# sile/libflate

Measured on AMD Instinct MI355X. Metric: gzip encode+decode throughput on 256 MiB synthetic text per GPU (uncompressed bytes through the round trip), higher is better.
Workload: dtype u8; 1 GPU; cfg2: gzip::Encoder (DefaultLz77Encoder, default options, mtime=0) + gzip::Decoder on TEXT(268435456 B) per GPU, write schedule S8K (8192-byte writes); bytes_per_gpu=268435456, schedule=S8K, compressed_bytes=129579521, parallelism=1 rank

## Files before the change

libflate_amd/csrc/lfx_api.cpp:

```cpp
#include "../../include/lfx.h"
#include "../../include/lfx_testhooks.h"

#include <hip/hip_runtime.h>

#include <algorithm>
#include <cstddef>
#include <cstdio>
#include <cstdlib>
#include <cstring>
#include <mutex>
#include <string>
#include <vector>

#include "lfx_ctx.h"
#include "lfx_device.h"
#include "lfx_huff.h"
#include "lfx_index.h"
#include "lfx_plan.h"
#include "lfx_abi_guard.h"

using namespace lfx;

static uint32_t host_crc32(const uint8_t *p, size_t n) {
    static uint32_t tab[256];
// ... 324 lines not shown
    hipStream_t st = c->stream;
    c->n_ev = 0;
    c->phase("start");
    for (const ChunkDesc &ch : plan.chunks)
        if (ch.len >= (1ull << 32) - 4) {
            c->set_error("an LZ77 chunk of 4 GiB or more is outside the reference's domain (u32 positions, default.rs:78)");
            return LFX_E_ARG;
        }
    const uint32_t nchunks = (uint32_t)plan.chunks.size(), nblocks = (uint32_t)plan.blocks.size();
    const bool match_v1 = c->force_match_v1 || c->diag.match_v1;
    if (c->force_match_v1 && !hc) c->match_fallbacks++;
    std::vector<SegDesc> segs;
    if (!hc) {
        uint64_t seg_len = SEG_POSITIONS;
        for (;;) {
            uint64_t cnt = 0;
            for (const ChunkDesc &ch : plan.chunks)
                if (!(ch.flags & CH_LITERALS) && ch.len > 3) cnt += div_up(ch.len - 3, seg_len);
            if (cnt >= 512 || seg_len <= 32768) break;
            seg_len /= 2;
        }
        for (uint32_t ci = 0; ci < nchunks; ci++) {
            const ChunkDesc &ch = plan.chunks[ci];
            if (ch.flags & CH_LITERALS) continue;
            for (uint64_t s = 0; s + 3 < ch.len; s += seg_len)
                segs.push_back(SegDesc{ci, (uint32_t)s, (uint32_t)std::min<uint64_t>(seg_len, ch.len - s), 0});
        }
    }
    uint64_t lnk_units = 0;
    for (SegDesc &sg : segs) {
        if (lnk_units > 0xFFFFFFFFull) { c->set_error("input too large for the link scratch"); return LFX_E_ARG; }
        sg.lnk_base = (uint32_t)lnk_units;
        lnk_units += div_up((uint64_t)sg.len + std::min<uint64_t>(sg.start, MAX_WINDOW) + 4, 64);
        lnk_units = (lnk_units + 1) & ~1ull;
    }
    std::vector<ParseWg> pwgs;
    for (uint32_t ci = 0; ci < nchunks && !hc; ci++) {
        const ChunkDesc &ch = plan.chunks[ci];
        if (ch.flags & CH_LITERALS) continue;
        for (uint32_t s = 0; s < ch.n_seg; s += PARSE_WG_SEGS) pwgs.push_back(ParseWg{ci, s});
    }
    if (pwgs.size() > 8) {
        const size_t nl = pwgs.size(), per = (nl + 7) / 8;
        std::vector<ParseWg> phys(per * 8);
        for (size_t i = 0; i < phys.size(); i++) {
            const size_t l = (i % 8) * per + i / 8;
            phys[i] = (i / 8 < per && l < nl && l / per == i % 8) ? pwgs[l] : ParseWg{0xFFFFFFFFu, 0u};
        }
        pwgs.swap(phys);
    }
    c->cur_nchunks = nchunks;
    c->cur_nblocks = nblocks;
    c->cur_ntiles = plan.n_tiles;
    c->cur_n = n;
    c->cur_in = d_in;
    int rc;
    if ((rc = c->d_chunks.reserve(sizeof(ChunkDesc) * std::max<size_t>(nchunks, 1)))) return rc;
    if ((rc = c->d_blocks.reserve(sizeof(BlockDesc) * std::max<size_t>(nblocks, 1)))) return rc;
    if ((rc = c->d_segs.reserve(sizeof(SegDesc) * std::max<size_t>(segs.size(), 1)))) return rc;
    if ((rc = c->d_pwgs.reserve(sizeof(ParseWg) * std::max<size_t>(pwgs.size(), 1)))) return rc;
    if (!hc && (rc = c->d_cd.reserve(2 * n + 64))) return rc;
    if (!hc && !match_v1 && (rc = c->d_glnk.reserve(264 * std::max<uint64_t>(lnk_units, 1)))) return rc;
    if (!hc && !match_v1 && (rc = c->d_ucount.reserve(4 * std::max<size_t>(segs.size(), 1)))) return rc;
    if (!hc && match_v1 && (rc = c->d_md.reserve(4 * std::max<uint64_t>(n, 1)))) return rc;
    if ((rc = c->d_codes.reserve(4 * std::max<uint64_t>(plan.n_codes_cap, 1)))) return rc;
    if ((rc = c->d_ncodes.reserve(4 * std::max<size_t>(nchunks, 1)))) return rc;
    if ((rc = c->d_vis.reserve(8 * std::max<uint64_t>(plan.n_vis, 1)))) return rc;
    if ((rc = c->d_segtmp.reserve(24ull * std::max<uint32_t>(plan.n_segs, 1)))) return rc;
    if (!hc && (rc = c->d_stage.reserve(4ull * (n + 64)))) return rc;
    if ((rc = c->d_chunkmap.reserve(4ull * (plan.n_tiles + plan.n_segs + 2)))) return rc;
    if ((rc = c->d_hist.reserve(4ull * 320 * std::max<size_t>(nblocks, 1)))) return rc;
    if ((rc = c->d_bc.reserve(sizeof(BlockCodes) * std::max<size_t>(nblocks, 1)))) return rc;
    if ((rc = c->d_block_start.reserve(8 * std::max<size_t>(nblocks, 1)))) return rc;
    if ((rc = c->d_tile_bits.reserve(4 * std::max<uint64_t>(plan.n_tiles, 1)))) return rc;
    if ((rc = c->d_tile_start.reserve(8 * std::max<uint64_t>(plan.n_tiles, 1)))) return rc;
    const uint64_t nspans = ck_nspans(n);
    if ((rc = c->d_ck.reserve(12 * nspans))) return rc;
    if ((rc = c->d_res.reserve(256))) return rc;
    if ((rc = c->d_small.reserve(70000))) return rc;

    auto upload = [&](int slot, DevBuf &b, const void *src, size_t bytes) -> hipError_t {
        std::vector<uint8_t> &sh = c->up_shadow[slot];
        const uint64_t tag = (uint64_t)(uintptr_t)b.p ^ ((uint64_t)b.gen << 48) ^ (1ull << 63);
        if (c->up_dev[slot] == tag && sh.size() == bytes && (bytes == 0 || memcmp(sh.data(), src, bytes) == 0)) return hipSuccess;
        sh.assign((const uint8_t *)src, (const uint8_t *)src + bytes);
        c->up_dev[slot] = tag;
        return bytes ? hipMemcpyAsync(b.p, sh.data(), bytes, hipMemcpyHostToDevice, st) : hipSuccess;
    };
    HIP_TRY(upload(0, c->d_chunks, plan.chunks.data(), sizeof(ChunkDesc) * nchunks));
    HIP_TRY(upload(1, c->d_blocks, plan.blocks.data(), sizeof(BlockDesc) * nblocks));
    HIP_TRY(upload(2, c->d_segs, segs.data(), sizeof(SegDesc) * segs.size()));
    HIP_TRY(upload(3, c->d_pwgs, pwgs.data(), sizeof(ParseWg) * pwgs.size()));
    const bool ucount_here = !hc && !match_v1 && !c->diag.match_v5;
    const ZeroSpan z_hist{(uint32_t *)c->d_hist.p, (uint32_t)(320 * std::max<size_t>(nblocks, 1))}, z_res{(uint32_t *)c->d_res.p, 64u},
        z_ucount{ucount_here ? (uint32_t *)c->d_ucount.p : nullptr, ucount_here ? (uint32_t)std::max<size_t>(segs.size(), 1) : 0u};
    c->phase("upload");
    uint32_t *tile_map = (uint32_t *)c->d_chunkmap.p, *seg_map = tile_map + plan.n_tiles;
    c->cur_tile_map = tile_map;
    if (int e_ = launch_chunk_maps(st, (const ChunkDesc *)c->d_chunks.p, nchunks, plan.n_tiles, plan.n_segs, tile_map, seg_map, z_hist,
                                   z_res, z_ucount)) {
        c->set_error(hipGetErrorString((hipError_t)e_));
        return LFX_E_DEVICE;
// ... 2 lines not shown
#define LAUNCH_TRY(call)                                                              \
    do {                                                                              \
        int e_ = (call);                                                              \
        if (e_) {                                                                     \
            c->set_error(std::string(#call) + ": " + hipGetErrorString((hipError_t)e_)); \
            return LFX_E_DEVICE;                                                      \
        }                                                                             \
    } while (0)

    uint64_t *mdbg = nullptr;
    if (c->diag.debug) mdbg = (uint64_t *)((uint8_t *)c->d_small.p + 32768);
    bool fused_hist = false;
    bool forked = false;
    uint32_t emit_per = 0, emit_parts = 0;
    if (hc) {
        if (hc->n_codes) HIP_TRY(hipMemcpyAsync(c->d_codes.p, hc->codes, 4ull * hc->n_codes, hipMemcpyHostToDevice, st));
        if (nchunks) HIP_TRY(hipMemcpyAsync(c->d_ncodes.p, hc->chunk_codes, 4ull * nchunks, hipMemcpyHostToDevice, st));
        c->phase("codes_upload");
    } else {
    uint32_t *d_match_flags = (uint32_t *)((uint8_t *)c->d_res.p + offsetof(EncodeResult, match_flags));
    uint16_t *d_cd = (uint16_t *)c->d_cd.p;
    if (match_v1) {
        LAUNCH_TRY(launch_match(st, d_in, n, (const ChunkDesc *)c->d_chunks.p, (const SegDesc *)c->d_segs.p,
                                (uint32_t)segs.size(), po.window_size, po.max_length, (uint32_t *)c->d_md.p, mdbg));
        LAUNCH_TRY(launch_md_to_cd(st, (const uint32_t *)c->d_md.p, n, d_cd));
    } else {
        if (!c->diag.match_v5) {
            const uint32_t ns = (uint32_t)segs.size();
            const uint32_t ncu = (uint32_t)std::max(c->n_cu, 1);
            const uint32_t want_parts = (uint32_t)std::max(c->diag.match_parts, 1);
            const uint32_t parts = ns >= 2 * ncu ? std::min<uint32_t>(std::min<uint32_t>(4, want_parts), ns / ncu) : 1;
            const SegDesc *dsegs = (const SegDesc *)c->d_segs.p;
            uint32_t *d_glnk = (uint32_t *)c->d_glnk.p;
            uint64_t *d_umask = (uint64_t *)((uint8_t *)c->d_glnk.p + 256 * std::max<uint64_t>(lnk_units, 1));
            uint32_t *d_ucount = (uint32_t *)c->d_ucount.p;
            for (uint32_t k = 0; k < parts; k++) {
                const uint32_t s0 = (uint32_t)((uint64_t)ns * k / parts), s1 = (uint32_t)((uint64_t)ns * (k + 1) / parts);
                LAUNCH_TRY(launch_match7(st, d_in, n, (const ChunkDesc *)c->d_chunks.p, dsegs + s0, s1 - s0, po.window_size, d_cd,
                                         d_glnk, d_umask, d_match_flags, k == 0 ? mdbg : nullptr));
                if (parts == 1 && c->timing_fine()) c->phase("lz77_cand");
                hipStream_t rs = parts > 1 ? c->side_stream : st;
                if (parts > 1) {
                    HIP_TRY(hipEventRecord(c->ev_part[k], st));
                    HIP_TRY(hipStreamWaitEvent(rs, c->ev_part[k], 0));
                }
                LAUNCH_TRY(launch_resolve7(rs, (const ChunkDesc *)c->d_chunks.p, dsegs + s0, s1 - s0, po.window_size, d_cd,
                                           d_glnk, d_umask, (uint32_t *)c->d_stage.p, d_ucount + s0, (uint32_t)std::max(c->diag.r7_cap, 0)));
            }
            if (parts > 1) {
                HIP_TRY(hipEventRecord(c->ev_res, c->side_stream));
                HIP_TRY(hipStreamWaitEvent(st, c->ev_res, 0));
            }
        }
        else
            LAUNCH_TRY(launch_match5(st, d_in, n, (const ChunkDesc *)c->d_chunks.p, (const SegDesc *)c->d_segs.p,
                                     (uint32_t)segs.size(), po.window_size, d_cd, (uint16_t *)c->d_glnk.p, d_match_flags, mdbg));
    }
    if (mdbg) {
        uint64_t hv[256];
        (void)hipMemcpy(hv, mdbg, sizeof hv, hipMemcpyDeviceToHost);
        const bool v5 = !match_v1 && c->diag.match_v5, v7 = !match_v1 && !c->diag.match_v5;
        if (v7) {
            for (int w = 0; w < 16; w++)
                fprintf(stderr, "[lfx] match7 wave%d: work=%llu barrier-wait=%llu tiles=%llu\n", w, (unsigned long long)hv[w * 8],
                        (unsigned long long)hv[w * 8 + 1], (unsigned long long)hv[w * 8 + 5]);
        } else {
            for (int w = 0; w < 16; w++)
                fprintf(stderr, "[lfx] match%s wave%d: %s=%llu %s=%llu wait=%llu tiles=%llu\n", match_v1 ? "1" : "5", w,
                        match_v1 ? "load" : "phaseA", (unsigned long long)hv[w * 8], match_v1 ? "work" : "phaseB",
                        (unsigned long long)hv[w * 8 + 1], (unsigned long long)hv[w * 8 + 2], (unsigned long long)hv[w * 8 + 5]);
        }
        if (v5) {
            uint64_t handed = 0;
            for (int w = 1; w < 16; w++) handed += hv[128 + w * 8 + 5];
            fprintf(stderr, "[lfx] match5 workgroup 0: %llu walks handed over to wave 0 of %llu positions; wave 0 waited %llu cycles for their loads\n",
                    (unsigned long long)handed, (unsigned long long)hv[5] * 960ull, (unsigned long long)hv[6]);
            for (int w = 1; w < 16; w++)
                fprintf(stderr, "[lfx] match5 wave%d loop trips: sum=%u max=%u tiles>4=%u tiles>8=%u\n", w, (unsigned)hv[w * 8 + 3],
                        (unsigned)(hv[w * 8 + 3] >> 32), (unsigned)hv[w * 8 + 4], (unsigned)(hv[w * 8 + 4] >> 32));
        }
// ... 1110 lines not shown
```

libflate_amd/csrc/lfx_common.h:

```cpp
#pragma once
#include <stdint.h>

#ifdef __HIPCC__
#define LFX_HD __host__ __device__
#else
#define LFX_HD
#endif

namespace lfx {

enum : uint32_t { BT_RAW = 0, BT_FIXED = 1, BT_DYNAMIC = 2 };

constexpr uint32_t MAX_WINDOW = 32768;
constexpr uint32_t MAX_LENGTH = 258;
constexpr uint32_t CODE_EOB = 0x01000000u;

struct ChunkDesc {
    uint64_t in_off;
    uint64_t len;
    uint64_t code_off;
    uint32_t block;
    uint32_t flags;
    uint64_t tile_base;
    uint64_t vis_base;
// ... 18 lines not shown
    uint32_t lit[288];
    uint32_t dist[32];
    uint64_t body_bits;
    uint32_t hdr_bits;
    uint32_t _pad;
    uint32_t hdr[160];
};

constexpr uint32_t PACK_TILE = 2048;
#ifndef LFX_PARSE_GROUP
#define LFX_PARSE_GROUP 52
#endif
constexpr uint32_t PARSE_GROUP = LFX_PARSE_GROUP;
constexpr uint32_t PARSE_SEG = 64 * PARSE_GROUP;
#ifndef LFX_PARSE_WG_SEGS
#define LFX_PARSE_WG_SEGS 12
#endif
constexpr uint32_t PARSE_WG_SEGS = LFX_PARSE_WG_SEGS;
#ifndef LFX_EMIT_WAVES
#define LFX_EMIT_WAVES 4
#endif
#ifndef LFX_EMIT_WG_PER_CU
#define LFX_EMIT_WG_PER_CU 16
#endif
constexpr uint32_t PARSE_EMIT_WAVES = LFX_EMIT_WAVES, PARSE_EMIT_WG_PER_CU = LFX_EMIT_WG_PER_CU;

#ifdef __HIPCC__
typedef const __attribute__((address_space(1))) uint32_t *gptr_u32;
typedef const __attribute__((address_space(1))) uint8_t *gptr_u8;
#endif

LFX_HD inline uint64_t div_up(uint64_t a, uint64_t b) { return (a + b - 1) / b; }

}
```

libflate_amd/csrc/lfx_device.h:

```cpp
#pragma once
#include <hip/hip_runtime.h>
#include <stdint.h>

#include "../../include/lfx.h"
#include "lfx_common.h"

namespace lfx {

struct SegDesc {
    uint32_t chunk;
    uint32_t start;
    uint32_t len;
    uint32_t lnk_base;
};
constexpr uint32_t SEG_POSITIONS = 256 * 1024;

struct EncodeResult {
    uint64_t end_bit;
    uint64_t out_bytes;
    uint32_t status;
    uint32_t crc32;
    uint32_t adler32;
    uint32_t match_flags;
};

struct BatchStream {
    uint64_t in_off, in_len;
    uint64_t out_off, out_cap;
    uint32_t first_block, n_blocks;
};

struct ParseWg {
    uint32_t chunk;
    uint32_t seg0;
};

int launch_match(hipStream_t st, const uint8_t *in, uint64_t in_bytes, const ChunkDesc *chunks,
                 const SegDesc *segs, uint32_t nsegs, uint32_t window, uint32_t max_len, uint32_t *md,
                 uint64_t *dbg = nullptr);
int launch_match7(hipStream_t st, const uint8_t *in, uint64_t in_bytes, const ChunkDesc *chunks, const SegDesc *segs,
                  uint32_t nsegs, uint32_t window, uint16_t *cd, uint32_t *glnk ,
                  uint64_t *umask , uint32_t *flags, uint64_t *dbg = nullptr);
int launch_resolve7(hipStream_t st, const ChunkDesc *chunks, const SegDesc *segs, uint32_t nsegs, uint32_t window, uint16_t *cd,
                    const uint32_t *glnk, const uint64_t *umask, uint32_t *ulist ,
                    uint32_t *ucount ,
                    uint32_t hop_cap = 0 );
int launch_match5(hipStream_t st, const uint8_t *in, uint64_t in_bytes, const ChunkDesc *chunks, const SegDesc *segs,
                  uint32_t nsegs, uint32_t window, uint16_t *cd, uint16_t *glnk, uint32_t *flags, uint64_t *dbg = nullptr);
int launch_md_to_cd(hipStream_t st, const uint32_t *md, uint64_t n, uint16_t *cd);
int launch_parse(hipStream_t st, const uint8_t *in, uint64_t in_bytes, const ChunkDesc *chunks, uint32_t nchunks,
                 uint32_t nsegs, const ParseWg *wgs, uint32_t nwgs, const uint16_t *cd, uint32_t max_len, uint64_t *vis,
                 uint32_t *seg_tmp, uint32_t *codes, uint32_t *ncodes, uint32_t *stage ,
                 const uint32_t *seg_map, int stop_after = 0 ,
                 uint64_t *dbg = nullptr ,
                 uint32_t *hist = nullptr ,
                 uint32_t emit_per = 0 ,
                 uint32_t emit_parts = 0 ,
                 hipEvent_t ev_walked = nullptr ,
                 const uint32_t *mflags = nullptr ,
                 int start_at = 0 );
struct ZeroSpan { uint32_t *p; uint32_t n; };
int launch_chunk_maps(hipStream_t st, const ChunkDesc *chunks, uint32_t nchunks, uint64_t ntiles, uint32_t nsegs,
                      uint32_t *tile_map, uint32_t *seg_map, ZeroSpan z0 = ZeroSpan{nullptr, 0}, ZeroSpan z1 = ZeroSpan{nullptr, 0},
                      ZeroSpan z2 = ZeroSpan{nullptr, 0});
int launch_histogram(hipStream_t st, const ChunkDesc *chunks, uint32_t nchunks, uint32_t split,
                     const uint32_t *codes, const uint32_t *ncodes, uint32_t *hist);
int launch_huffman(hipStream_t st, const BlockDesc *blocks, uint32_t nblocks, const uint32_t *hist,
                   BlockCodes *bc, uint64_t *dbg = nullptr);
int launch_offsets(hipStream_t st, const BlockDesc *blocks, uint32_t nblocks, const BlockCodes *bc,
                   uint64_t start_bit, uint64_t cap_bits, uint64_t *block_start, EncodeResult *res);
int launch_offsets_batch(hipStream_t st, const BatchStream *streams, uint32_t count, const BlockDesc *blocks, const BlockCodes *bc,
                         uint32_t hdr_len, uint32_t trailer_len, uint64_t *block_start, uint64_t *stream_end, int32_t *status,
                         EncodeResult *res);
int launch_frame_batch(hipStream_t st, int format, const BatchStream *streams, uint32_t count, const uint8_t *hdr, uint32_t hdr_len,
                       const uint64_t *stream_end, const uint32_t *crc, const uint32_t *adler, const EncodeResult *res, uint32_t *out,
                       uint64_t *out_len);
struct MembersGeom {
    uint64_t n, member_size;
// ... 31 lines not shown
```

libflate_amd/csrc/lfx_match7.hip:

```cpp
#include <hip/hip_runtime.h>
#include <stdint.h>
#include <stdlib.h>

#include <type_traits>

#include "lfx_common.h"
#include "lfx_device.h"

namespace lfx {
namespace m7 {

constexpr int THREADS = 1024;
constexpr uint32_t NG = 14;
constexpr uint32_t TILE = NG * 64;
constexpr uint64_t ROLE_IDX = 0x6564325104321000ull;
constexpr uint32_t ROLE_IS_P = 0x227Cu;
constexpr uint32_t ROLE_IS_C = 0xDD80u;
#ifndef LFX_M7_PRIO
#define LFX_M7_PRIO 0xa2a2800fu
#endif
constexpr int AHEAD = 4;
#ifndef LFX_M7_BARRIER
#define LFX_M7_BARRIER 1
#endif
constexpr uint32_t NP = 7, NC = 7;
#ifndef LFX_M7_EXP
#define LFX_M7_EXP 0
#endif
constexpr uint32_t RQ_SAME_PREV = 1u << 30, RQ_NEXT_SAME = 1u << 31, RQ_ADDR_BITS = 18;
constexpr uint32_t BUCKET_BITS = 14, TAG_BITS = 24 - BUCKET_BITS;
constexpr uint32_t TAG_MASK = (1u << TAG_BITS) - 1;
constexpr uint32_t KEY_MULT = 0x00374ADDu;
constexpr uint32_t SPOS0 = MAX_WINDOW + 1;
constexpr uint32_t UNRES = 0x8000u;

constexpr uint32_t OFF_DUMMY = 0;
constexpr uint32_t OFF_TAB = 128;
constexpr uint32_t OFF_DUMMY2 = OFF_TAB + (4u << BUCKET_BITS);
constexpr uint32_t OFF_SEC = OFF_DUMMY2 + 128;
constexpr uint32_t SEC_DELTA = OFF_SEC - OFF_TAB;
constexpr uint32_t OFF_CTL = OFF_SEC + (4u << BUCKET_BITS);
constexpr uint32_t OFF_RQ = OFF_CTL + 64;
constexpr uint32_t OFF_R1 = OFF_RQ + 4 * TILE * 4;
constexpr uint32_t OFF_R2 = OFF_R1 + 3 * TILE * 4;
constexpr uint32_t LDS_BYTES = OFF_R2 + 2 * TILE * 4;
static_assert(LDS_BYTES <= 160 * 1024, "LDS budget");
static_assert(OFF_DUMMY + SEC_DELTA == OFF_DUMMY2, "a dummy request's second entry is a dummy too");
static_assert(LDS_BYTES < (1u << RQ_ADDR_BITS) && TAG_BITS + RQ_ADDR_BITS <= 30, "LDS addresses fit the request, below its two run bits");
static_assert(SEG_POSITIONS + MAX_WINDOW + SPOS0 + 8 * TILE < (1u << (32 - TAG_BITS)), "segment-relative positions fit the entry");
static_assert(KEY_MULT < (1u << 24) && (KEY_MULT & 1), "24-bit multiplication, bijective");
static_assert(NG == 14 && NP + NC == NG, "operand lists below: two batches of seven; two groups per helper wavefront");
static_assert(TILE % 4 == 0, "a lane's byte phase is the same in every tile");

__device__ __forceinline__ void lds_barrier() { asm volatile("s_waitcnt lgkmcnt(0)\n\ts_barrier" ::: "memory"); }
__device__ __forceinline__ void ctr_set(uint32_t a, int v) { asm volatile("ds_write_b32 %0, %1" ::"v"(a), "v"(v) : "memory"); }
__device__ __forceinline__ void ctr_wait(uint32_t a, uint32_t n, int v) {
    const uint32_t l = threadIdx.x & 63;
    const uint32_t mine = a + (l < n ? l : 0u) * 4;
    for (;;) {
        int got;
        asm volatile("ds_read_b32 %0, %1\n\ts_waitcnt lgkmcnt(0)" : "=v"(got) : "v"(mine) : "memory");
        if (__ballot(got - v < 0) == 0) break;
        __builtin_amdgcn_s_sleep(1);
    }
}

__device__ __forceinline__ void xchg7(uint32_t (&old)[14], const uint32_t (&addr)[14], const uint32_t (&val)[14], const int o) {
    asm volatile(
        "ds_wrxchg_rtn_b32 %0, %7, %14\n\t"
        "ds_wrxchg_rtn_b32 %1, %8, %15\n\t"
        "ds_wrxchg_rtn_b32 %2, %9, %16\n\t"
        "ds_wrxchg_rtn_b32 %3, %10, %17\n\t"
        "ds_wrxchg_rtn_b32 %4, %11, %18\n\t"
        "ds_wrxchg_rtn_b32 %5, %12, %19\n\t"
        "ds_wrxchg_rtn_b32 %6, %13, %20"
        : "=&v"(old[o]), "=&v"(old[o + 1]), "=&v"(old[o + 2]), "=&v"(old[o + 3]), "=&v"(old[o + 4]), "=&v"(old[o + 5]), "=&v"(old[o + 6])
        : "v"(addr[o]), "v"(addr[o + 1]), "v"(addr[o + 2]), "v"(addr[o + 3]), "v"(addr[o + 4]), "v"(addr[o + 5]), "v"(addr[o + 6]),
          "v"(val[o]), "v"(val[o + 1]), "v"(val[o + 2]), "v"(val[o + 3]), "v"(val[o + 4]), "v"(val[o + 5]), "v"(val[o + 6])
        : "memory");
}
__device__ __forceinline__ void mskor7(uint32_t (&old)[14], const uint32_t (&addr)[14], const uint32_t (&mask)[14],
                                       const uint32_t (&val)[14], const int o) {
    asm volatile(
        "ds_mskor_rtn_b32 %0, %7, %14, %21 \n\t"
        "ds_mskor_rtn_b32 %1, %8, %15, %22 \n\t"
        "ds_mskor_rtn_b32 %2, %9, %16, %23 \n\t"
        "ds_mskor_rtn_b32 %3, %10, %17, %24 \n\t"
        "ds_mskor_rtn_b32 %4, %11, %18, %25 \n\t"
        "ds_mskor_rtn_b32 %5, %12, %19, %26 \n\t"
        "ds_mskor_rtn_b32 %6, %13, %20, %27"
        : "=&v"(old[o]), "=&v"(old[o + 1]), "=&v"(old[o + 2]), "=&v"(old[o + 3]), "=&v"(old[o + 4]), "=&v"(old[o + 5]), "=&v"(old[o + 6])
        : "v"(addr[o]), "v"(addr[o + 1]), "v"(addr[o + 2]), "v"(addr[o + 3]), "v"(addr[o + 4]), "v"(addr[o + 5]), "v"(addr[o + 6]),
          "v"(mask[o]), "v"(mask[o + 1]), "v"(mask[o + 2]), "v"(mask[o + 3]), "v"(mask[o + 4]), "v"(mask[o + 5]), "v"(mask[o + 6]),
          "v"(val[o]), "v"(val[o + 1]), "v"(val[o + 2]), "v"(val[o + 3]), "v"(val[o + 4]), "v"(val[o + 5]), "v"(val[o + 6])
        : "memory");
}
__device__ __forceinline__ void lds_wait14(uint32_t (&v)[14]) {
    asm volatile("s_waitcnt lgkmcnt(0)"
                 : "+v"(v[0]), "+v"(v[1]), "+v"(v[2]), "+v"(v[3]), "+v"(v[4]), "+v"(v[5]), "+v"(v[6]), "+v"(v[7]), "+v"(v[8]),
                   "+v"(v[9]), "+v"(v[10]), "+v"(v[11]), "+v"(v[12]), "+v"(v[13])
                 :
                 : "memory");
}

}

template <bool DBG>
__global__ __launch_bounds__(m7::THREADS) void lz77_match7_kernel(
    const uint8_t *__restrict__ in, uint64_t in_bytes, const ChunkDesc *__restrict__ chunks,
    const SegDesc *__restrict__ segs, uint32_t window, uint16_t *__restrict__ cd,
    uint32_t *__restrict__ glnk, uint64_t *__restrict__ umask, uint32_t *__restrict__ flags, uint64_t *__restrict__ dbg) {
    using namespace m7;
    __shared__ __attribute__((aligned(16))) unsigned char smem[LDS_BYTES];
    uint32_t *rqb = (uint32_t *)(smem + OFF_RQ);
    uint32_t *r1b = (uint32_t *)(smem + OFF_R1);
    uint32_t *r2b = (uint32_t *)(smem + OFF_R2);
    const uint32_t lds0 = (uint32_t)(uintptr_t)(__attribute__((address_space(3))) unsigned char *)smem;

    const SegDesc sg = segs[blockIdx.x];
    const ChunkDesc ch = chunks[sg.chunk];
    const uint32_t tid = threadIdx.x, lane = tid & 63;
    const uint32_t wave = (uint32_t)__builtin_amdgcn_readfirstlane((int)(tid >> 6));
    const uint32_t n = (uint32_t)ch.len;
    if (ch.flags & CH_LITERALS) return;
    const uint32_t end = (n > 3 ? n : 3) - 3;
    const uint32_t q0 = sg.start;
    const uint32_t q1 = min(sg.start + sg.len, end);
    if (q0 >= q1) return;
    const uint32_t l0 = q0 > MAX_WINDOW ? q0 - MAX_WINDOW : 0;
    const uint32_t base = l0 & ~3u;
    const int ntiles = (int)((q1 - base + TILE - 1) / TILE);

    const int i_first = -1 - AHEAD;
    const int n_iter = (ntiles + 2 - i_first + AHEAD - 1) / AHEAD * AHEAD;
    const int i_end = i_first + n_iter;

    {
        uint4 *t4 = (uint4 *)smem;
        for (uint32_t i = tid; i < (OFF_RQ >> 4); i += THREADS) t4[i] = make_uint4(0, 0, 0, 0);
    }
    lds_barrier();
    bool runs_mode;
    {
        const uint64_t a0 = (uint64_t)(in + ch.in_off);
// ... 65 lines not shown
                    asm("v_mul_u32_u24 %0, %1, %2" : "=v"(kk) : "v"(key), "s"(KEY_MULT));
                    uint32_t r = ((((kk >> TAG_BITS) & ((1u << BUCKET_BITS) - 1)) * 4u + tab) << TAG_BITS) | (kk & TAG_MASK);
                    if (!interior) {
                        const uint32_t p = t0 + hidx + g * 64;
                        r = (p >= l0 && p < q1) ? r : dummy;
                    }
                    if (RUNS && __ballot(((key ^ (key >> 8)) & 0xFFFFu) == 0)) {
                        const uint32_t below = (uint32_t)__shfl_up((int)r, 1), above = (uint32_t)__shfl_down((int)r, 1);
                        const bool sp = lane > 0 && below == r && r != dummy, ns = lane < 63 && above == r && r != dummy;
                        r |= (sp ? RQ_SAME_PREV : 0u) | (ns ? RQ_NEXT_SAME : 0u);
                    }
                    rq[g * 64] = r;
                }
                if (!LFX_M7_BARRIER) ctr_set(c_p + 4 * ridx, tp + 1);
            }
            {
                const uint32_t toff = (uint32_t)(i + 1 + AHEAD) * TILE;
                const uint32_t off = off_lane + toff;
                if (((base + shift) & ~3u) + toff + TILE + 72 <= last_off && last_off >= TILE + 72) {
                    ld[0] = ldw(off); ld[1] = ldw(off + 4); ld[2] = ldw(off + 64); ld[3] = ldw(off + 68);
                } else {
                    ld[0] = ldw(min(off, last_off)); ld[1] = ldw(min(off + 4, last_off));
                    ld[2] = ldw(min(off + 64, last_off)); ld[3] = ldw(min(off + 68, last_off));
                }
            }
            sync(c0);
        };
        static_assert(AHEAD == 4, "register sets below");
        for (int i = i_first; i < i_end; i += 4) { p_iter(i, ldA); p_iter(i + 1, ldB); p_iter(i + 2, ldC); p_iter(i + 3, ldD); }
    } else if ((ROLE_IS_C >> wave) & 1) {
        const uint32_t hidx = ridx * 128 + lane;
        uint8_t *glnk_b = (uint8_t *)(glnk + (uint64_t)sg.lnk_base * 64u);
        uint8_t *cd_b = (uint8_t *)(cd + ch.in_off + base);
        uint64_t *um_s = umask + sg.lnk_base;
        int32_t dmin = 1;
        auto c_iter = [&](int i) {
            const uint64_t c0 = DBG ? clock64() : 0;
            const int tc = i - 2;
            if (tc >= 0 && tc < ntiles) {
                wait_for(c_x2, 1, tc + 1);
                const uint32_t t0 = base + (uint32_t)tc * TILE;
                const bool interior = t0 >= q0 && t0 + TILE <= q1;
                uint32_t rq[2], o1[2], o2[2];
#pragma unroll
                for (uint32_t g = 0; g < 2; ++g) {
                    rq[g] = rqb[(uint32_t)(tc & 3) * TILE + hidx + g * 64];
                    o1[g] = r1b[(uint32_t)(tc % 3) * TILE + hidx + g * 64];
                    o2[g] = r2b[(uint32_t)(tc & 1) * TILE + hidx + g * 64];
                }
                if (!LFX_M7_BARRIER) {
                    asm volatile("s_waitcnt lgkmcnt(0)" : "+v"(rq[0]), "+v"(rq[1]), "+v"(o1[0]), "+v"(o1[1]), "+v"(o2[0]), "+v"(o2[1]));
                    ctr_set(c_c + 4 * ridx, tc + 1);
                }
                const uint32_t rel = (uint32_t)tc * TILE + hidx;
                const uint32_t boff = rel * 2;
                uint64_t um[2] = {0, 0};
                bool has_act[2] = {true, true};
#pragma unroll
                for (uint32_t g = 0; g < 2; ++g) {
                    const uint32_t sp = rel + g * 64 + SPOS0;
                    const uint32_t d1 = sp - (o1[g] >> TAG_BITS), d2 = sp - (o2[g] >> TAG_BITS);
                    const bool same1 = ((o1[g] ^ rq[g]) & TAG_MASK) == 0, same2 = ((o2[g] ^ rq[g]) & TAG_MASK) == 0;
                    const uint32_t dl = same1 ? d2 : d1;
                    const uint32_t lnk = dl <= MAX_WINDOW ? dl : 0u;
                    uint32_t a2 = same2 ? d2 : d2 + (UNRES - 1);
                    a2 = d2 > window ? 0u : a2;
                    const uint32_t a1 = same1 ? d1 : a2;
                    const uint32_t ans = d1 > window ? 0u : a1;
                    if (interior) {
                        dmin = min(dmin, min((int32_t)d1, (int32_t)d2));
                        if (!(LFX_M7_EXP & 1)) *(uint32_t *)(glnk_b + 2 * boff + g * 256) = lnk | (rq[g] << 16);
                        if (!(LFX_M7_EXP & 2)) *(uint16_t *)(cd_b + boff + g * 128) = (uint16_t)ans;
                        um[g] = __ballot(ans > UNRES);
                    } else {
                        const uint32_t p = t0 + hidx + g * 64;
                        const bool valid = p >= l0 && p < q1, act = valid && p >= q0;
                        if (valid) dmin = min(dmin, min((int32_t)d1, (int32_t)d2));
                        if (valid) *(uint32_t *)(glnk_b + 2 * boff + g * 256) = lnk | (rq[g] << 16);
                        if (act) *(uint16_t *)(cd_b + boff + g * 128) = (uint16_t)ans;
                        um[g] = __ballot(act && ans > UNRES);
                        has_act[g] = __ballot(act) != 0;
                    }
                }
                if (lane == 0) {
                    if (has_act[0] && has_act[1]) *(ulonglong2 *)(um_s + (rel >> 6)) = make_ulonglong2(um[0], um[1]);
                    else if (has_act[0]) um_s[rel >> 6] = um[0];
                    else if (has_act[1]) um_s[(rel >> 6) + 1] = um[1];
                }
            }
            sync(c0);
        };
        for (int i = i_first; i < i_end; ++i) c_iter(i);
        if (__ballot(dmin <= 0) && lane == 0) atomicOr(flags, 1u);
    } else if (wave == 0) {
        for (int i = i_first; i < i_end; ++i) {
            const uint64_t c0 = DBG ? clock64() : 0;
            if (i >= 0 && i < ntiles) {
                wait_for(c_p, NP, i + 1);
                wait_for(c_c, NC, i - 2);
                const uint32_t *rq = rqb + (uint32_t)(i & 3) * TILE + lane;
                uint32_t *r1 = r1b + (uint32_t)(i % 3) * TILE + lane;
                const uint32_t ent0 = ((uint32_t)i * TILE + lane + SPOS0) << TAG_BITS;
                uint32_t q[NG], ad[NG], vl[NG], od[NG];
#pragma unroll
                for (uint32_t s = 0; s < NG; ++s) q[s] = rq[s * 64];
                constexpr bool runs = RUNS;
                const uint32_t dummy_a = lds0 + OFF_DUMMY + (lane & 31) * 4;
#pragma unroll
                for (uint32_t s = 0; s < NG; ++s) {
                    ad[s] = __builtin_amdgcn_ubfe(q[s], TAG_BITS, RQ_ADDR_BITS);
                    vl[s] = (q[s] & TAG_MASK) | (ent0 + ((s * 64u) << TAG_BITS));
                }
                if constexpr (runs) {
#pragma unroll
                    for (uint32_t s = 0; s < NG; ++s) ad[s] = (q[s] >> 30) == 3u ? dummy_a : ad[s];
                }
                xchg7(od, ad, vl, 0);
                xchg7(od, ad, vl, 7);
                lds_wait14(od);
                if constexpr (runs) {
#pragma unroll
// ... 24 lines not shown
                for (uint32_t s = 0; s < NG; ++s) {
                    const bool differ = ((q[s] ^ o[s]) & TAG_MASK) != 0;
                    ad[s] = __builtin_amdgcn_ubfe(q[s], TAG_BITS, RQ_ADDR_BITS) + SEC_DELTA;
                    mk[s] = differ ? 0xFFFFFFFFu : 0u;
                    vl[s] = differ ? o[s] : 0u;
                }
                if constexpr (runs) {
#pragma unroll
                    for (uint32_t s = 0; s < NG; ++s) ad[s] = (q[s] & RQ_SAME_PREV) ? dummy_a : ad[s];
                }
                mskor7(od, ad, mk, vl, 0);
                mskor7(od, ad, mk, vl, 7);
                lds_wait14(od);
                if constexpr (runs) {
#pragma unroll
                    for (uint32_t s = 0; s < NG; ++s) {
                        const bool sp = (q[s] & RQ_SAME_PREV) != 0;
                        const uint64_t heads = __ballot(!sp) & ((2ull << lane) - 1ull);
                        const uint32_t h = 63u - (uint32_t)__builtin_clzll(heads);
                        const uint32_t behind = mk[s] ? o[s] : od[s];
                        const uint32_t fromhead = (uint32_t)__shfl((int)behind, (int)h);
                        od[s] = sp ? fromhead : od[s];
                    }
                }
#pragma unroll
                for (uint32_t s = 0; s < NG; ++s) r2[s * 64] = od[s];
                if (!LFX_M7_BARRIER) ctr_set(c_x2, t2 + 1);
            }
            sync(c0);
        }
    }
    };
    if (runs_mode) pipeline(std::true_type{}); else pipeline(std::false_type{});
    if (DBG && dbg && blockIdx.x == 0 && lane == 0) {
        uint64_t *d = dbg + wave * 8;
        d[0] = cy_work; d[1] = cy_wait; d[2] = 0; d[3] = 0; d[4] = 0; d[5] = (uint64_t)ntiles; d[6] = 0; d[7] = 0;
    }
}

namespace r7 {
constexpr uint32_t SLAB_WORDS = 128;
constexpr uint32_t SLABS = SEG_POSITIONS / 64 / SLAB_WORDS;
constexpr uint32_t THREADS = 256, WGS = 2, NS = 4;
}

__global__ __launch_bounds__(r7::SLAB_WORDS) void lz77_compact7_kernel(
    const ChunkDesc *__restrict__ chunks, const SegDesc *__restrict__ segs, const uint64_t *__restrict__ umask,
    uint32_t *__restrict__ ulist, uint32_t *__restrict__ ucount) {
    using namespace r7;
    __shared__ uint32_t wsum[2], gbase;
    const uint32_t seg = blockIdx.x / (SLABS + 1), slab = blockIdx.x % (SLABS + 1);
    const SegDesc sg = segs[seg];
    if (slab * (SLAB_WORDS * 64) >= sg.len + 64) return;
    const ChunkDesc ch = chunks[sg.chunk];
    const uint32_t n = (uint32_t)ch.len;
    const uint32_t end = (n > 3 ? n : 3) - 3;
    const uint32_t q0 = sg.start, q1 = min(sg.start + sg.len, end);
    if (q0 >= q1) return;
    const uint32_t l0 = q0 > MAX_WINDOW ? q0 - MAX_WINDOW : 0;
    const uint32_t base = l0 & ~3u;
    const uint32_t w = (q0 - base) / 64 + slab * SLAB_WORDS + threadIdx.x;
    const uint32_t p0 = base + w * 64;
    uint64_t m = 0;
    if (p0 < q1) m = umask[sg.lnk_base + w];
    if (base + (w - threadIdx.x) * 64 >= q1) return;
    const uint32_t c = (uint32_t)__popcll(m);
    uint32_t x = c;
    for (int o = 1; o < 64; o <<= 1) { const uint32_t y = __shfl_up((int)x, o); if ((threadIdx.x & 63) >= (uint32_t)o) x += y; }
    if ((threadIdx.x & 63) == 63) wsum[threadIdx.x >> 6] = x;
    __syncthreads();
    const uint32_t total = wsum[0] + wsum[1];
    if (total == 0) return;
    if (threadIdx.x == 0) gbase = atomicAdd(&ucount[seg], total);
    __syncthreads();
    uint32_t at = gbase + (x - c) + ((threadIdx.x >> 6) ? wsum[0] : 0u);
    uint32_t *ul = ulist + ch.in_off + sg.start;
    while (m) {
        const uint32_t b = (uint32_t)__builtin_ctzll(m);
        m &= m - 1;
        ul[at++] = p0 + b;
    }
}

__global__ __launch_bounds__(r7::THREADS) void lz77_resolve7_kernel(
    const ChunkDesc *__restrict__ chunks, const SegDesc *__restrict__ segs, uint32_t window, uint16_t *__restrict__ cd,
    const uint32_t *__restrict__ glnk, const uint32_t *__restrict__ ulist, const uint32_t *__restrict__ ucount,
    uint32_t hop_cap ) {
    using namespace r7;
    const uint32_t seg = blockIdx.x / WGS, part = blockIdx.x % WGS;
    const uint32_t total = ucount[seg];
    if (part * THREADS >= total) return;
    const SegDesc sg = segs[seg];
    const ChunkDesc ch = chunks[sg.chunk];
    const uint32_t q0 = sg.start;
    const uint32_t l0 = q0 > MAX_WINDOW ? q0 - MAX_WINDOW : 0;
    const uint32_t base = l0 & ~3u;
    uint16_t *cd_c = cd + ch.in_off;
    const uint32_t *glnk_s = glnk + (uint64_t)sg.lnk_base * 64u;
    const uint32_t *ulist_s = ulist + ch.in_off + sg.start;
    constexpr uint32_t STRIDE = WGS * THREADS;
    uint32_t state[NS], i[NS], p[NS], tag[NS], r[NS], dist[NS], hops[NS];
    bool first[NS];
#pragma unroll
    for (uint32_t j = 0; j < NS; ++j) {
        i[j] = part * THREADS + threadIdx.x + j * STRIDE;
        state[j] = i[j] < total ? 0u : 3u;
        p[j] = tag[j] = r[j] = dist[j] = hops[j] = 0;
        first[j] = false;
    }
    for (;;) {
        bool any = false;
#pragma unroll
        for (uint32_t j = 0; j < NS; ++j) any |= state[j] != 3u;
        if (!__ballot(any)) break;
        uint32_t e[NS], c[NS], rec[NS];
#pragma unroll
        for (uint32_t j = 0; j < NS; ++j) {
            const bool s0 = state[j] == 0, s1 = state[j] == 1, s2 = state[j] == 2;
            e[j] = c[j] = rec[j] = 0;
            if (s0) e[j] = ulist_s[i[j]];
            if (s1) c[j] = cd_c[p[j]];
            if (s1 || s2) rec[j] = glnk_s[(s1 ? p[j] : r[j]) - base];
        }
#pragma unroll
        for (uint32_t j = 0; j < NS; ++j) asm volatile("" : "+v"(e[j]), "+v"(c[j]), "+v"(rec[j]));
#pragma unroll
        for (uint32_t j = 0; j < NS; ++j) {
            if (state[j] == 0) { p[j] = e[j]; state[j] = 1; }
            else if (state[j] == 1) {
                tag[j] = rec[j] >> 16;
                dist[j] = c[j] - m7::UNRES + 1;
                r[j] = p[j] - dist[j];
                first[j] = true;
                hops[j] = 0;
                state[j] = 2;
            } else if (state[j] == 2) {
                bool done = false;
                uint32_t ans = 0;
                const uint32_t l = rec[j] & 0xFFFFu;
                if (!first[j] && (rec[j] >> 16) == tag[j]) { done = true; ans = dist[j]; }
                else {
                    dist[j] += l;
                    if (l == 0 || dist[j] > window) done = true;
                    else r[j] -= l;
                    if (hop_cap && ++hops[j] >= hop_cap) done = true;
                }
                first[j] = false;
                if (done) {
                    cd_c[p[j]] = (uint16_t)ans;
                    i[j] += NS * STRIDE;
                    state[j] = i[j] < total ? 0u : 3u;
                }
            }
        }
    }
}

int launch_match7(hipStream_t st, const uint8_t *in, uint64_t in_bytes, const ChunkDesc *chunks, const SegDesc *segs,
                  uint32_t nsegs, uint32_t window, uint16_t *cd, uint32_t *glnk, uint64_t *umask, uint32_t *flags, uint64_t *dbg) {
    if (nsegs == 0) return 0;
    if (dbg)
        hipLaunchKernelGGL(lz77_match7_kernel<true>, dim3(nsegs), dim3(m7::THREADS), 0, st, in, in_bytes, chunks, segs, window,
                           cd, glnk, umask, flags, dbg);
    else
        hipLaunchKernelGGL(lz77_match7_kernel<false>, dim3(nsegs), dim3(m7::THREADS), 0, st, in, in_bytes, chunks, segs, window,
                           cd, glnk, umask, flags, dbg);
    const hipError_t e_ = hipGetLastError();
    return e_ != hipSuccess ? (int)e_ : 0;
}

int launch_resolve7(hipStream_t st, const ChunkDesc *chunks, const SegDesc *segs, uint32_t nsegs, uint32_t window, uint16_t *cd,
                    const uint32_t *glnk, const uint64_t *umask, uint32_t *ulist, uint32_t *ucount, uint32_t hop_cap) {
    if (nsegs == 0) return 0;
    hipLaunchKernelGGL(lz77_compact7_kernel, dim3(nsegs * (r7::SLABS + 1)), dim3(r7::SLAB_WORDS), 0, st, chunks, segs, umask, ulist,
                       ucount);
    hipError_t e_ = hipGetLastError();
    if (e_ != hipSuccess) return (int)e_;
    hipLaunchKernelGGL(lz77_resolve7_kernel, dim3(nsegs * r7::WGS), dim3(r7::THREADS), 0, st, chunks, segs, window, cd, glnk, ulist,
                       ucount, hop_cap);
    e_ = hipGetLastError();
    return e_ != hipSuccess ? (int)e_ : 0;
}

}
```

Measured before the change: 59.22 GB/s.

## Emit unresolved-match list directly from match kernel, drop compaction pass

The match kernel now appends each unresolved position to a per-segment list, using an LDS atomic counter plus wave ballot and mbcnt prefix. Each entry is packed with its relative position, tag and second-candidate distance. This removes the bitmask write and the separate compact kernel launch. The resolve kernel starts chains straight from the packed entry instead of re-reading cd and glnk for the head record. The cost is a larger staging buffer (8 bytes per position), an atomic per tile in the match kernel, and list order no longer being positional, which may hurt locality in resolve.

```diff
diff --git a/libflate_amd/csrc/lfx_api.cpp b/libflate_amd/csrc/lfx_api.cpp
--- a/libflate_amd/csrc/lfx_api.cpp
+++ b/libflate_amd/csrc/lfx_api.cpp
@@ -380,7 +380,6 @@
         if (lnk_units > 0xFFFFFFFFull) { c->set_error("input too large for the link scratch"); return LFX_E_ARG; }
         sg.lnk_base = (uint32_t)lnk_units;
         lnk_units += div_up((uint64_t)sg.len + std::min<uint64_t>(sg.start, MAX_WINDOW) + 4, 64);
-        lnk_units = (lnk_units + 1) & ~1ull;
     }
     std::vector<ParseWg> pwgs;
     for (uint32_t ci = 0; ci < nchunks && !hc; ci++) {
@@ -408,14 +407,14 @@
     if ((rc = c->d_segs.reserve(sizeof(SegDesc) * std::max<size_t>(segs.size(), 1)))) return rc;
     if ((rc = c->d_pwgs.reserve(sizeof(ParseWg) * std::max<size_t>(pwgs.size(), 1)))) return rc;
     if (!hc && (rc = c->d_cd.reserve(2 * n + 64))) return rc;
-    if (!hc && !match_v1 && (rc = c->d_glnk.reserve(264 * std::max<uint64_t>(lnk_units, 1)))) return rc;
+    if (!hc && !match_v1 && (rc = c->d_glnk.reserve(256 * std::max<uint64_t>(lnk_units, 1)))) return rc;
     if (!hc && !match_v1 && (rc = c->d_ucount.reserve(4 * std::max<size_t>(segs.size(), 1)))) return rc;
     if (!hc && match_v1 && (rc = c->d_md.reserve(4 * std::max<uint64_t>(n, 1)))) return rc;
     if ((rc = c->d_codes.reserve(4 * std::max<uint64_t>(plan.n_codes_cap, 1)))) return rc;
     if ((rc = c->d_ncodes.reserve(4 * std::max<size_t>(nchunks, 1)))) return rc;
     if ((rc = c->d_vis.reserve(8 * std::max<uint64_t>(plan.n_vis, 1)))) return rc;
     if ((rc = c->d_segtmp.reserve(24ull * std::max<uint32_t>(plan.n_segs, 1)))) return rc;
-    if (!hc && (rc = c->d_stage.reserve(4ull * (n + 64)))) return rc;
+    if (!hc && (rc = c->d_stage.reserve((match_v1 || c->diag.match_v5 ? 4ull : 8ull) * (n + 64)))) return rc;
     if ((rc = c->d_chunkmap.reserve(4ull * (plan.n_tiles + plan.n_segs + 2)))) return rc;
     if ((rc = c->d_hist.reserve(4ull * 320 * std::max<size_t>(nblocks, 1)))) return rc;
     if ((rc = c->d_bc.reserve(sizeof(BlockCodes) * std::max<size_t>(nblocks, 1)))) return rc;
@@ -484,12 +483,12 @@
             const uint32_t parts = ns >= 2 * ncu ? std::min<uint32_t>(std::min<uint32_t>(4, want_parts), ns / ncu) : 1;
             const SegDesc *dsegs = (const SegDesc *)c->d_segs.p;
             uint32_t *d_glnk = (uint32_t *)c->d_glnk.p;
-            uint64_t *d_umask = (uint64_t *)((uint8_t *)c->d_glnk.p + 256 * std::max<uint64_t>(lnk_units, 1));
+            UlEntry *d_ulist = (UlEntry *)c->d_stage.p;
             uint32_t *d_ucount = (uint32_t *)c->d_ucount.p;
             for (uint32_t k = 0; k < parts; k++) {
                 const uint32_t s0 = (uint32_t)((uint64_t)ns * k / parts), s1 = (uint32_t)((uint64_t)ns * (k + 1) / parts);
                 LAUNCH_TRY(launch_match7(st, d_in, n, (const ChunkDesc *)c->d_chunks.p, dsegs + s0, s1 - s0, po.window_size, d_cd,
-                                         d_glnk, d_umask, d_match_flags, k == 0 ? mdbg : nullptr));
+                                         d_glnk, d_ulist, d_ucount + s0, d_match_flags, k == 0 ? mdbg : nullptr));
                 if (parts == 1 && c->timing_fine()) c->phase("lz77_cand");
                 hipStream_t rs = parts > 1 ? c->side_stream : st;
                 if (parts > 1) {
@@ -497,7 +496,7 @@
                     HIP_TRY(hipStreamWaitEvent(rs, c->ev_part[k], 0));
                 }
                 LAUNCH_TRY(launch_resolve7(rs, (const ChunkDesc *)c->d_chunks.p, dsegs + s0, s1 - s0, po.window_size, d_cd,
-                                           d_glnk, d_umask, (uint32_t *)c->d_stage.p, d_ucount + s0, (uint32_t)std::max(c->diag.r7_cap, 0)));
+                                           d_glnk, d_ulist, d_ucount + s0, (uint32_t)std::max(c->diag.r7_cap, 0)));
             }
             if (parts > 1) {
                 HIP_TRY(hipEventRecord(c->ev_res, c->side_stream));
diff --git a/libflate_amd/csrc/lfx_common.h b/libflate_amd/csrc/lfx_common.h
--- a/libflate_amd/csrc/lfx_common.h
+++ b/libflate_amd/csrc/lfx_common.h
@@ -74,4 +74,11 @@
 
 LFX_HD inline uint64_t div_up(uint64_t a, uint64_t b) { return (a + b - 1) / b; }
 
+constexpr uint32_t UL_REL_BITS = 19, UL_TAG_BITS = 10, UL_D2_BITS = 15;
+struct UlEntry { uint32_t lo, hi; };
+LFX_HD inline UlEntry ul_pack(uint32_t rel, uint32_t tag, uint32_t d2) { return UlEntry{rel | (tag << UL_REL_BITS), d2 - 1}; }
+LFX_HD inline uint32_t ul_rel(UlEntry e) { return e.lo & ((1u << UL_REL_BITS) - 1); }
+LFX_HD inline uint32_t ul_tag(UlEntry e) { return (e.lo >> UL_REL_BITS) & ((1u << UL_TAG_BITS) - 1); }
+LFX_HD inline uint32_t ul_d2(UlEntry e) { return (e.hi & ((1u << UL_D2_BITS) - 1)) + 1; }
+
 }
diff --git a/libflate_amd/csrc/lfx_device.h b/libflate_amd/csrc/lfx_device.h
--- a/libflate_amd/csrc/lfx_device.h
+++ b/libflate_amd/csrc/lfx_device.h
@@ -40,10 +40,11 @@
                  uint64_t *dbg = nullptr);
 int launch_match7(hipStream_t st, const uint8_t *in, uint64_t in_bytes, const ChunkDesc *chunks, const SegDesc *segs,
                   uint32_t nsegs, uint32_t window, uint16_t *cd, uint32_t *glnk ,
-                  uint64_t *umask , uint32_t *flags, uint64_t *dbg = nullptr);
+                  UlEntry *ulist ,
+                  uint32_t *ucount ,
+                  uint32_t *flags, uint64_t *dbg = nullptr);
 int launch_resolve7(hipStream_t st, const ChunkDesc *chunks, const SegDesc *segs, uint32_t nsegs, uint32_t window, uint16_t *cd,
-                    const uint32_t *glnk, const uint64_t *umask, uint32_t *ulist ,
-                    uint32_t *ucount ,
+                    const uint32_t *glnk, const UlEntry *ulist, const uint32_t *ucount,
                     uint32_t hop_cap = 0 );
 int launch_match5(hipStream_t st, const uint8_t *in, uint64_t in_bytes, const ChunkDesc *chunks, const SegDesc *segs,
                   uint32_t nsegs, uint32_t window, uint16_t *cd, uint16_t *glnk, uint32_t *flags, uint64_t *dbg = nullptr);
diff --git a/libflate_amd/csrc/lfx_match7.hip b/libflate_amd/csrc/lfx_match7.hip
--- a/libflate_amd/csrc/lfx_match7.hip
+++ b/libflate_amd/csrc/lfx_match7.hip
@@ -40,7 +40,8 @@
 constexpr uint32_t OFF_SEC = OFF_DUMMY2 + 128;
 constexpr uint32_t SEC_DELTA = OFF_SEC - OFF_TAB;
 constexpr uint32_t OFF_CTL = OFF_SEC + (4u << BUCKET_BITS);
-constexpr uint32_t OFF_RQ = OFF_CTL + 64;
+constexpr uint32_t OFF_UCNT = OFF_CTL + 64;
+constexpr uint32_t OFF_RQ = OFF_UCNT + 64;
 constexpr uint32_t OFF_R1 = OFF_RQ + 4 * TILE * 4;
 constexpr uint32_t OFF_R2 = OFF_R1 + 3 * TILE * 4;
 constexpr uint32_t LDS_BYTES = OFF_R2 + 2 * TILE * 4;
@@ -51,6 +52,8 @@
 static_assert(KEY_MULT < (1u << 24) && (KEY_MULT & 1), "24-bit multiplication, bijective");
 static_assert(NG == 14 && NP + NC == NG, "operand lists below: two batches of seven; two groups per helper wavefront");
 static_assert(TILE % 4 == 0, "a lane's byte phase is the same in every tile");
+static_assert(SEG_POSITIONS + MAX_WINDOW + 4 <= (1u << UL_REL_BITS) && TAG_BITS == UL_TAG_BITS && MAX_WINDOW <= (1u << UL_D2_BITS),
+              "a list entry holds the position, the tag and d2");
 
 __device__ __forceinline__ void lds_barrier() { asm volatile("s_waitcnt lgkmcnt(0)\n\ts_barrier" ::: "memory"); }
 __device__ __forceinline__ void ctr_set(uint32_t a, int v) { asm volatile("ds_write_b32 %0, %1" ::"v"(a), "v"(v) : "memory"); }
@@ -109,7 +112,8 @@
 __global__ __launch_bounds__(m7::THREADS) void lz77_match7_kernel(
     const uint8_t *__restrict__ in, uint64_t in_bytes, const ChunkDesc *__restrict__ chunks,
     const SegDesc *__restrict__ segs, uint32_t window, uint16_t *__restrict__ cd,
-    uint32_t *__restrict__ glnk, uint64_t *__restrict__ umask, uint32_t *__restrict__ flags, uint64_t *__restrict__ dbg) {
+    uint32_t *__restrict__ glnk, UlEntry *__restrict__ ulist, uint32_t *__restrict__ ucount, uint32_t *__restrict__ flags,
+    uint64_t *__restrict__ dbg) {
     using namespace m7;
     __shared__ __attribute__((aligned(16))) unsigned char smem[LDS_BYTES];
     uint32_t *rqb = (uint32_t *)(smem + OFF_RQ);
@@ -241,7 +245,8 @@
         const uint32_t hidx = ridx * 128 + lane;
         uint8_t *glnk_b = (uint8_t *)(glnk + (uint64_t)sg.lnk_base * 64u);
         uint8_t *cd_b = (uint8_t *)(cd + ch.in_off + base);
-        uint64_t *um_s = umask + sg.lnk_base;
+        uint2 *ul_s = (uint2 *)ulist + ch.in_off + sg.start;
+        uint32_t *ucnt = (uint32_t *)(smem + OFF_UCNT);
         int32_t dmin = 1;
         auto c_iter = [&](int i) {
             const uint64_t c0 = DBG ? clock64() : 0;
@@ -263,39 +268,50 @@
                 }
                 const uint32_t rel = (uint32_t)tc * TILE + hidx;
                 const uint32_t boff = rel * 2;
-                uint64_t um[2] = {0, 0};
-                bool has_act[2] = {true, true};
-#pragma unroll
-                for (uint32_t g = 0; g < 2; ++g) {
-                    const uint32_t sp = rel + g * 64 + SPOS0;
-                    const uint32_t d1 = sp - (o1[g] >> TAG_BITS), d2 = sp - (o2[g] >> TAG_BITS);
-                    const bool same1 = ((o1[g] ^ rq[g]) & TAG_MASK) == 0, same2 = ((o2[g] ^ rq[g]) & TAG_MASK) == 0;
-                    const uint32_t dl = same1 ? d2 : d1;
-                    const uint32_t lnk = dl <= MAX_WINDOW ? dl : 0u;
-                    uint32_t a2 = same2 ? d2 : d2 + (UNRES - 1);
-                    a2 = d2 > window ? 0u : a2;
-                    const uint32_t a1 = same1 ? d1 : a2;
-                    const uint32_t ans = d1 > window ? 0u : a1;
-                    if (interior) {
-                        dmin = min(dmin, min((int32_t)d1, (int32_t)d2));
-                        if (!(LFX_M7_EXP & 1)) *(uint32_t *)(glnk_b + 2 * boff + g * 256) = lnk | (rq[g] << 16);
-                        if (!(LFX_M7_EXP & 2)) *(uint16_t *)(cd_b + boff + g * 128) = (uint16_t)ans;
-                        um[g] = __ballot(ans > UNRES);
-                    } else {
-                        const uint32_t p = t0 + hidx + g * 64;
-                        const bool valid = p >= l0 && p < q1, act = valid && p >= q0;
-                        if (valid) dmin = min(dmin, min((int32_t)d1, (int32_t)d2));
-                        if (valid) *(uint32_t *)(glnk_b + 2 * boff + g * 256) = lnk | (rq[g] << 16);
-                        if (act) *(uint16_t *)(cd_b + boff + g * 128) = (uint16_t)ans;
-                        um[g] = __ballot(act && ans > UNRES);
-                        has_act[g] = __ballot(act) != 0;
+                auto body = [&](auto interior_tag) {
+                    constexpr bool INTERIOR = decltype(interior_tag)::value;
+                    uint32_t lnk[2], ans[2], dd2[2];
+                    bool valid[2] = {true, true}, act[2] = {true, true};
+#pragma unroll
+                    for (uint32_t g = 0; g < 2; ++g) {
+                        const uint32_t sp = rel + g * 64 + SPOS0;
+                        const uint32_t d1 = sp - (o1[g] >> TAG_BITS), d2 = sp - (o2[g] >> TAG_BITS);
+                        const bool same1 = ((o1[g] ^ rq[g]) & TAG_MASK) == 0, same2 = ((o2[g] ^ rq[g]) & TAG_MASK) == 0;
+                        const uint32_t dl = same1 ? d2 : d1;
+                        lnk[g] = dl <= MAX_WINDOW ? dl : 0u;
+                        uint32_t a2 = same2 ? d2 : d2 + (UNRES - 1);
+                        a2 = d2 > window ? 0u : a2;
+                        const uint32_t a1 = same1 ? d1 : a2;
+                        ans[g] = d1 > window ? 0u : a1;
+                        dd2[g] = d2;
+                        if (!INTERIOR) {
+                            const uint32_t p = t0 + hidx + g * 64;
+                            valid[g] = p >= l0 && p < q1;
+                            act[g] = valid[g] && p >= q0;
+                        }
+                        if (valid[g]) dmin = min(dmin, min((int32_t)d1, (int32_t)d2));
                     }
-                }
-                if (lane == 0) {
-                    if (has_act[0] && has_act[1]) *(ulonglong2 *)(um_s + (rel >> 6)) = make_ulonglong2(um[0], um[1]);
-                    else if (has_act[0]) um_s[rel >> 6] = um[0];
-                    else if (has_act[1]) um_s[(rel >> 6) + 1] = um[1];
-                }
+                    const bool open0 = act[0] && ans[0] > UNRES, open1 = act[1] && ans[1] > UNRES;
+                    const uint64_t m0 = __ballot(open0), m1 = __ballot(open1);
+                    const bool any_open = (m0 | m1) != 0;
+                    uint32_t at = 0;
+                    if (any_open && lane == 0) at = atomicAdd(ucnt, (uint32_t)__popcll(m0) + (uint32_t)__popcll(m1));
+#pragma unroll
+                    for (uint32_t g = 0; g < 2; ++g) {
+                        if (valid[g] && !(INTERIOR && (LFX_M7_EXP & 1))) *(uint32_t *)(glnk_b + 2 * boff + g * 256) = lnk[g] | (rq[g] << 16);
+                        if (act[g] && !(INTERIOR && (LFX_M7_EXP & 2))) *(uint16_t *)(cd_b + boff + g * 128) = (uint16_t)ans[g];
+                    }
+                    if (any_open) {
+                        at = (uint32_t)__builtin_amdgcn_readfirstlane((int)at);
+                        const UlEntry e0 = ul_pack(rel, rq[0] & TAG_MASK, dd2[0]), e1 = ul_pack(rel + 64, rq[1] & TAG_MASK, dd2[1]);
+                        const uint32_t i0 = at + __builtin_amdgcn_mbcnt_hi((uint32_t)(m0 >> 32), __builtin_amdgcn_mbcnt_lo((uint32_t)m0, 0u));
+                        const uint32_t i1 = at + (uint32_t)__popcll(m0) +
+                                            __builtin_amdgcn_mbcnt_hi((uint32_t)(m1 >> 32), __builtin_amdgcn_mbcnt_lo((uint32_t)m1, 0u));
+                        if (open0) ul_s[i0] = make_uint2(e0.lo, e0.hi);
+                        if (open1) ul_s[i1] = make_uint2(e1.lo, e1.hi);
+                    }
+                };
+                if (interior) body(std::true_type{}); else body(std::false_type{});
             }
             sync(c0);
         };
@@ -386,6 +402,8 @@
     }
     };
     if (runs_mode) pipeline(std::true_type{}); else pipeline(std::false_type{});
+    lds_barrier();
+    if (tid == 0) ucount[blockIdx.x] = *(const uint32_t *)(smem + OFF_UCNT);
     if (DBG && dbg && blockIdx.x == 0 && lane == 0) {
         uint64_t *d = dbg + wave * 8;
         d[0] = cy_work; d[1] = cy_wait; d[2] = 0; d[3] = 0; d[4] = 0; d[5] = (uint64_t)ntiles; d[6] = 0; d[7] = 0;
@@ -393,9 +411,9 @@
 }
 
 namespace r7 {
+constexpr uint32_t THREADS = 256, WGS = 2, NS = 4;
 constexpr uint32_t SLAB_WORDS = 128;
 constexpr uint32_t SLABS = SEG_POSITIONS / 64 / SLAB_WORDS;
-constexpr uint32_t THREADS = 256, WGS = 2, NS = 4;
 }
 
 __global__ __launch_bounds__(r7::SLAB_WORDS) void lz77_compact7_kernel(
@@ -438,7 +456,7 @@
 
 __global__ __launch_bounds__(r7::THREADS) void lz77_resolve7_kernel(
     const ChunkDesc *__restrict__ chunks, const SegDesc *__restrict__ segs, uint32_t window, uint16_t *__restrict__ cd,
-    const uint32_t *__restrict__ glnk, const uint32_t *__restrict__ ulist, const uint32_t *__restrict__ ucount,
+    const uint32_t *__restrict__ glnk, const UlEntry *__restrict__ ulist, const uint32_t *__restrict__ ucount,
     uint32_t hop_cap ) {
     using namespace r7;
     const uint32_t seg = blockIdx.x / WGS, part = blockIdx.x % WGS;
@@ -449,50 +467,60 @@
     const uint32_t q0 = sg.start;
     const uint32_t l0 = q0 > MAX_WINDOW ? q0 - MAX_WINDOW : 0;
     const uint32_t base = l0 & ~3u;
-    uint16_t *cd_c = cd + ch.in_off;
+    uint16_t *cd_s = cd + ch.in_off + base;
     const uint32_t *glnk_s = glnk + (uint64_t)sg.lnk_base * 64u;
-    const uint32_t *ulist_s = ulist + ch.in_off + sg.start;
+    const uint2 *ulist_s = (const uint2 *)ulist + ch.in_off + sg.start;
     constexpr uint32_t STRIDE = WGS * THREADS;
-    uint32_t state[NS], i[NS], p[NS], tag[NS], r[NS], dist[NS], hops[NS];
-    bool first[NS];
+    uint32_t i[NS], rel[NS], tag[NS], r[NS], dist[NS], hops[NS];
+    uint2 nx[NS];
+    bool live[NS], first[NS], want[NS];
+    auto begin = [&](uint32_t j) {
+        const UlEntry e{nx[j].x, nx[j].y};
+        rel[j] = ul_rel(e);
+        tag[j] = ul_tag(e);
+        dist[j] = ul_d2(e);
+        r[j] = rel[j] - dist[j];
+        first[j] = true;
+        hops[j] = 0;
+        i[j] += NS * STRIDE;
+        want[j] = i[j] < total;
+    };
 #pragma unroll
     for (uint32_t j = 0; j < NS; ++j) {
         i[j] = part * THREADS + threadIdx.x + j * STRIDE;
-        state[j] = i[j] < total ? 0u : 3u;
-        p[j] = tag[j] = r[j] = dist[j] = hops[j] = 0;
-        first[j] = false;
-    }
+        live[j] = i[j] < total;
+        nx[j] = make_uint2(0, 0);
+        rel[j] = tag[j] = r[j] = dist[j] = hops[j] = 0;
+        first[j] = want[j] = false;
+        if (live[j]) nx[j] = ulist_s[i[j]];
+    }
+#pragma unroll
+    for (uint32_t j = 0; j < NS; ++j) asm volatile("" : "+v"(nx[j].x), "+v"(nx[j].y));
+#pragma unroll
+    for (uint32_t j = 0; j < NS; ++j)
+        if (live[j]) begin(j);
     for (;;) {
         bool any = false;
 #pragma unroll
-        for (uint32_t j = 0; j < NS; ++j) any |= state[j] != 3u;
+        for (uint32_t j = 0; j < NS; ++j) any |= live[j];
         if (!__ballot(any)) break;
-        uint32_t e[NS], c[NS], rec[NS];
+        uint32_t rec[NS];
 #pragma unroll
         for (uint32_t j = 0; j < NS; ++j) {
-            const bool s0 = state[j] == 0, s1 = state[j] == 1, s2 = state[j] == 2;
-            e[j] = c[j] = rec[j] = 0;
-            if (s0) e[j] = ulist_s[i[j]];
-            if (s1) c[j] = cd_c[p[j]];
-            if (s1 || s2) rec[j] = glnk_s[(s1 ? p[j] : r[j]) - base];
+            rec[j] = 0;
+            if (live[j]) rec[j] = glnk_s[r[j]];
+            if (want[j]) nx[j] = ulist_s[i[j]];
+            want[j] = false;
         }
 #pragma unroll
-        for (uint32_t j = 0; j < NS; ++j) asm volatile("" : "+v"(e[j]), "+v"(c[j]), "+v"(rec[j]));
+        for (uint32_t j = 0; j < NS; ++j) asm volatile("" : "+v"(rec[j]), "+v"(nx[j].x), "+v"(nx[j].y));
 #pragma unroll
         for (uint32_t j = 0; j < NS; ++j) {
-            if (state[j] == 0) { p[j] = e[j]; state[j] = 1; }
-            else if (state[j] == 1) {
-                tag[j] = rec[j] >> 16;
-                dist[j] = c[j] - m7::UNRES + 1;
-                r[j] = p[j] - dist[j];
-                first[j] = true;
-                hops[j] = 0;
-                state[j] = 2;
-            } else if (state[j] == 2) {
+            if (live[j]) {
                 bool done = false;
                 uint32_t ans = 0;
                 const uint32_t l = rec[j] & 0xFFFFu;
-                if (!first[j] && (rec[j] >> 16) == tag[j]) { done = true; ans = dist[j]; }
+                if (!first[j] && ((rec[j] >> 16) & m7::TAG_MASK) == tag[j]) { done = true; ans = dist[j]; }
                 else {
                     dist[j] += l;
                     if (l == 0 || dist[j] > window) done = true;
@@ -501,9 +529,9 @@
                 }
                 first[j] = false;
                 if (done) {
-                    cd_c[p[j]] = (uint16_t)ans;
-                    i[j] += NS * STRIDE;
-                    state[j] = i[j] < total ? 0u : 3u;
+                    cd_s[rel[j]] = (uint16_t)ans;
+                    live[j] = i[j] < total;
+                    if (live[j]) begin(j);
                 }
             }
         }
@@ -511,28 +539,25 @@
 }
 
 int launch_match7(hipStream_t st, const uint8_t *in, uint64_t in_bytes, const ChunkDesc *chunks, const SegDesc *segs,
-                  uint32_t nsegs, uint32_t window, uint16_t *cd, uint32_t *glnk, uint64_t *umask, uint32_t *flags, uint64_t *dbg) {
+                  uint32_t nsegs, uint32_t window, uint16_t *cd, uint32_t *glnk, UlEntry *ulist, uint32_t *ucount, uint32_t *flags,
+                  uint64_t *dbg) {
     if (nsegs == 0) return 0;
     if (dbg)
         hipLaunchKernelGGL(lz77_match7_kernel<true>, dim3(nsegs), dim3(m7::THREADS), 0, st, in, in_bytes, chunks, segs, window,
-                           cd, glnk, umask, flags, dbg);
+                           cd, glnk, ulist, ucount, flags, dbg);
     else
         hipLaunchKernelGGL(lz77_match7_kernel<false>, dim3(nsegs), dim3(m7::THREADS), 0, st, in, in_bytes, chunks, segs, window,
-                           cd, glnk, umask, flags, dbg);
+                           cd, glnk, ulist, ucount, flags, dbg);
     const hipError_t e_ = hipGetLastError();
     return e_ != hipSuccess ? (int)e_ : 0;
 }
 
 int launch_resolve7(hipStream_t st, const ChunkDesc *chunks, const SegDesc *segs, uint32_t nsegs, uint32_t window, uint16_t *cd,
-                    const uint32_t *glnk, const uint64_t *umask, uint32_t *ulist, uint32_t *ucount, uint32_t hop_cap) {
+                    const uint32_t *glnk, const UlEntry *ulist, const uint32_t *ucount, uint32_t hop_cap) {
     if (nsegs == 0) return 0;
-    hipLaunchKernelGGL(lz77_compact7_kernel, dim3(nsegs * (r7::SLABS + 1)), dim3(r7::SLAB_WORDS), 0, st, chunks, segs, umask, ulist,
-                       ucount);
-    hipError_t e_ = hipGetLastError();
-    if (e_ != hipSuccess) return (int)e_;
     hipLaunchKernelGGL(lz77_resolve7_kernel, dim3(nsegs * r7::WGS), dim3(r7::THREADS), 0, st, chunks, segs, window, cd, glnk, ulist,
                        ucount, hop_cap);
-    e_ = hipGetLastError();
+    const hipError_t e_ = hipGetLastError();
     return e_ != hipSuccess ? (int)e_ : 0;
 }
 
```

Result: no change. 59.73 GB/s (median of 6 runs) (+0.9%).
